# kyutai-labs/moshi

Hardware: AMD Instinct MI355X
Metric: 12.5 Hz frames/s end-to-end Mimi+Moshi-7B (higher is better)
Workload: dtype bf16

## Files before the change

### include/moshi_mi.h

```cpp
#ifndef MOSHI_MI_H_
#define MOSHI_MI_H_

#include <stdint.h>

#ifdef __cplusplus
extern "C" {
#endif

#define MMI_ABI_VERSION 3

typedef enum mmi_status {
    MMI_OK = 0,
    MMI_ERR_INVALID = -1,
    MMI_ERR_SHAPE = -2,
    MMI_ERR_STATE = -3,
    MMI_ERR_HIP = -4,
    MMI_ERR_MISSING_WEIGHT = -5,
    MMI_ERR_UNSUPPORTED = -6,
    MMI_ERR_BUSY = -7,
    MMI_ERR_NO_CHANNEL = -8
} mmi_status;

typedef enum mmi_dtype { MMI_F32 = 0, MMI_BF16 = 1, MMI_I64 = 2, MMI_F16 = 3, MMI_I8 = 4, MMI_F8E4M3 = 5 ,
                         MMI_F4E2M1X2 = 6 ,
// ... 195 lines not shown
};
typedef struct mmi_tts_script mmi_tts_script;
int mmi_lm_set_row_script(mmi_lm* lm, int32_t session, const mmi_tts_script* script, mmi_stream stream);
struct mmi_tts_status {
    int32_t has_script, end_step, n_consumed;
    int32_t* consumption_times;
    int32_t capacity;
};
typedef struct mmi_tts_status mmi_tts_status;
int mmi_lm_row_script_status(mmi_lm* lm, int32_t session, mmi_tts_status* out, mmi_stream stream);

int mmi_lm_step(mmi_lm* lm, const int64_t* user_codes, int32_t n_user, int64_t* out_tokens,
                float* opt_text_logits, float* opt_audio_logits, const float* opt_noise, int32_t batch,
                int32_t* valid, mmi_stream stream);

int mmi_lm_set_phase_callback(mmi_lm* lm, int (*fn)(void* user, mmi_stream stream), void* user);

typedef struct mmi_lm_hooks {
    int (*on_text_logits)(void* user);
    int (*on_text_token)(void* user);
    int (*on_audio_tokens)(void* user);
    void* user;
} mmi_lm_hooks;
int mmi_lm_set_hooks(mmi_lm* lm, const mmi_lm_hooks* hooks_or_null);
int mmi_lm_hook_io(mmi_lm* lm, int32_t which, int32_t write, void* buf, int64_t nbytes, mmi_stream stream);
int32_t mmi_lm_has_hooks(const mmi_lm* lm);

int mmi_lm_force_next_tokens(mmi_lm* lm, const int64_t* tokens, mmi_stream stream);

int mmi_lm_set_hidden_taps(mmi_lm* lm, int32_t on);
// ... 74 lines not shown
```

### moshi_amd/_capi.py

```python
from __future__ import annotations

import ctypes as C
import os
from pathlib import Path
from typing import Dict, Optional, Sequence

import torch

_PKG = Path(__file__).resolve().parent
DEFAULT_LIB = _PKG / "libmoshi_mi.so"

MMI_OK, MMI_ERR_INVALID, MMI_ERR_SHAPE, MMI_ERR_STATE, MMI_ERR_HIP, MMI_ERR_MISSING_WEIGHT, MMI_ERR_UNSUPPORTED, MMI_ERR_BUSY, \
    MMI_ERR_NO_CHANNEL = 0, -1, -2, -3, -4, -5, -6, -7, -8
MMI_F32, MMI_BF16, MMI_I64, MMI_F16, MMI_I8, MMI_F8E4M3, MMI_F4E2M1X2, MMI_E8M0 = 0, 1, 2, 3, 4, 5, 6, 7

_DTYPES = {torch.float32: MMI_F32, torch.bfloat16: MMI_BF16, torch.int64: MMI_I64, torch.float16: MMI_F16,
           torch.int8: MMI_I8, torch.float8_e4m3fn: MMI_F8E4M3, torch.uint8: MMI_F4E2M1X2}
MXFP4_SCALE_SUFFIX = ".weight_scale_e8m0"


class TensorDesc(C.Structure):
    _fields_ = [("name", C.c_char_p), ("data", C.c_void_p), ("dtype", C.c_int32), ("ndim", C.c_int32),
                ("shape", C.c_int64 * 4)]

# ... 135 lines not shown
    "mmi_lm_streaming_stop": (C.c_int, [_P]),
    "mmi_lm_set_exec_mask": (C.c_int, [_P, _P, _P]),
    "mmi_lm_reset": (C.c_int, [_P, _P, _P]),
    "mmi_row_sampling_check": (C.c_int, [C.POINTER(RowSampling)]),
    "mmi_lm_set_row_sampling": (C.c_int, [_P, _P, C.POINTER(RowSampling), _P]),
    "mmi_lm_clear_row_sampling": (C.c_int, [_P, _P, _P]),
    "mmi_lm_set_text_end_padding_id": (C.c_int, [_P, C.c_int32]),
    "mmi_lm_set_cross_capacity": (C.c_int, [_P, C.c_int32]),
    "mmi_lm_cross_capacity": (C.c_int, [_P]),
    "mmi_lm_set_row_condition": (C.c_int, [_P, C.c_int32, C.POINTER(RowCondition), _P]),
    "mmi_lm_enable_tts_machine": (C.c_int, [_P, C.POINTER(TTSParams), C.c_int32, C.c_int32, C.c_int32]),
    "mmi_lm_set_row_script": (C.c_int, [_P, C.c_int32, C.POINTER(TTSScriptC), _P]),
    "mmi_lm_row_script_status": (C.c_int, [_P, C.c_int32, C.POINTER(TTSStatus), _P]),
    "mmi_lm_step": (C.c_int, [_P, _P, C.c_int32, _P, _P, _P, _P, C.c_int32, C.POINTER(C.c_int32), _P]),
    "mmi_lm_force_next_tokens": (C.c_int, [_P, _P, _P]),
    "mmi_lm_set_phase_callback": (C.c_int, [_P, _P, _P]),
    "mmi_lm_set_hooks": (C.c_int, [_P, C.POINTER(LMHooks)]),
    "mmi_lm_hook_io": (C.c_int, [_P, C.c_int32, C.c_int32, _P, C.c_int64, _P]),
    "mmi_mimi_get_cfg": (C.c_int, [_P, C.POINTER(MimiCfg)]),
    "mmi_lm_get_cfg": (C.c_int, [_P, C.POINTER(LMCfg)]),
    "mmi_batcher_create": (C.c_int, [_P, _P, C.POINTER(BatcherCfg), C.POINTER(_P)]),
    "mmi_batcher_destroy": (None, [_P]),
    "mmi_batcher_open": (C.c_int, [_P, C.POINTER(C.c_int64)]),
    "mmi_batcher_open_with": (C.c_int, [_P, C.POINTER(RowSampling), C.POINTER(C.c_int64)]),
    "mmi_batcher_open_cond": (C.c_int, [_P, C.POINTER(RowSampling), C.POINTER(BatcherCondition), C.POINTER(C.c_int64)]),
    "mmi_batcher_close": (C.c_int, [_P, C.c_int64]),
    "mmi_batcher_push_pcm": (C.c_int, [_P, C.c_int64, _P, C.c_int32]),
    "mmi_batcher_step": (C.c_int, [_P, C.POINTER(C.c_int32)]),
    "mmi_batcher_pop": (C.c_int, [_P, C.c_int64, _P, _P, C.POINTER(C.c_int32)]),
    "mmi_batcher_get_stats": (C.c_int, [_P, C.POINTER(BatcherStats)]),
# ... 1 lines not shown
    "mmi_lm_launch_list": (C.c_int64, [_P, _P, C.c_int64]),
    "mmi_mimi_launch_list": (C.c_int64, [_P, C.c_int32, _P, C.c_int64]),
    "mmi_lm_seek": (C.c_int, [_P, _P, _P]),
    "mmi_lm_profile_begin": (C.c_int, [_P]),
    "mmi_lm_profile_sites": (C.c_int64, [_P, _P, C.c_int64]),
    "mmi_lm_profile_end": (C.c_int, [_P, C.POINTER(C.c_double), C.POINTER(C.c_int64), C.POINTER(C.c_int64),
                                     C.POINTER(C.c_char_p)]),
}


_SINCE_ROW_SAMPLING = ("mmi_row_sampling_check", "mmi_lm_set_row_sampling", "mmi_lm_clear_row_sampling", "mmi_batcher_open_with",
                       "mmi_lm_set_text_end_padding_id")
_SINCE_ROW_CONDITION = ("mmi_lm_set_cross_capacity", "mmi_lm_cross_capacity", "mmi_lm_set_row_condition", "mmi_batcher_open_cond")
_SINCE_TTS_MACHINE = ("mmi_lm_enable_tts_machine", "mmi_lm_set_row_script", "mmi_lm_row_script_status")
_SINCE_MANY_ROWS = ("mmi_lm_create_rows",)


def _missing(name, path):
    what = ("handles above 64 model rows" if name in _SINCE_MANY_ROWS else
            "the TTS script machine" if name in _SINCE_TTS_MACHINE else
            "per-session conditions" if name in _SINCE_ROW_CONDITION else "per-session sampling")

    def refuse(*_a):
        raise RuntimeError(f"{path} does not export {name}: it was built before {what} existed")
    return refuse


class Lib:

    def __init__(self, path: Path):
        self.path = Path(path)
        self.cdll = C.CDLL(str(self.path))
        for name, (res, args) in SIGNATURES.items():
            if name in _SINCE_ROW_SAMPLING + _SINCE_ROW_CONDITION + _SINCE_TTS_MACHINE + _SINCE_MANY_ROWS and not hasattr(self.cdll, name):
                setattr(self, name, _missing(name, self.path))
                continue
            fn = getattr(self.cdll, name)
            fn.restype = res
            fn.argtypes = args
            setattr(self, name, fn)

    def last_error(self) -> str:
        msg = self.mmi_last_error()
        return msg.decode() if msg else ""

    def check(self, rc: int) -> None:
        if rc == MMI_OK:
            return
        msg = f"{self.last_error()} (mmi status {rc})"
# ... 90 lines not shown
```

### moshi_amd/csrc/duplex.hip

```cpp
#include "mmi_common.h"

namespace {

__global__ void k_flag_publish(long* flag, long v) { mmi_flag_publish(flag, v); }
__global__ void k_flag_wait(const long* flag, long v) {
    if (threadIdx.x == 0) mmi_flag_wait(flag, v);
}

enum { S_IN = 0, S_ENC0, S_ENC1, S_WAIT0, S_WAIT1, S_LM0, S_PHASE, S_LM1, S_DEC0, S_DEC1, S_COUNT };
__global__ void k_stamp(long* p) { *p = mmi_wall_clock(); }
__global__ void k_flag_wait_stamped(const long* flag, long v, long* p) {
    if (threadIdx.x == 0) {
        p[0] = mmi_wall_clock();
        mmi_flag_wait(flag, v);
        p[1] = mmi_wall_clock();
    }
}

struct Pending { bool live = false, valid = false; float* pcm_out = nullptr; int64_t* tokens_out = nullptr; long frame = 0; };

enum { F_ENC = 0, F_LM = 1, F_DEC = 2, F_IN = 3, F_COUNT = 4 };

}

// ... 126 lines not shown
    } else {
        MMI_HIP_CHECK(hipStreamCreateWithFlags(&d->sL, hipStreamNonBlocking));
        MMI_HIP_CHECK(hipStreamCreateWithFlags(&d->sE, hipStreamNonBlocking));
        MMI_HIP_CHECK(hipStreamCreateWithFlags(&d->sD, hipStreamNonBlocking));
    }
    for (int i = 0; i < 2; ++i) {
        MMI_HIP_CHECK(hipEventCreateWithFlags(&d->ev_lm[i], hipEventDisableTiming));
        MMI_HIP_CHECK(hipEventCreateWithFlags(&d->ev_phase[i], hipEventDisableTiming));
        MMI_HIP_CHECK(hipMalloc((void**)&d->codes[i], (size_t)d->B * d->K * sizeof(int64_t)));
    }
    for (int i = 0; i < 3; ++i) {
        MMI_HIP_CHECK(hipEventCreateWithFlags(&d->ev_dec[i], hipEventDisableTiming));
        MMI_HIP_CHECK(hipMalloc((void**)&d->tokens[i], (size_t)d->B * d->NTOK * sizeof(int64_t)));
    }
    for (int i = 0; i < d->in_slots; ++i) MMI_HIP_CHECK(hipMalloc((void**)&d->pcm_in[i], (size_t)d->B * d->F * sizeof(float)));
    return MMI_OK;
}

int enqueue_decode(mmi_duplex* d, int p, bool host_saw_step) {
    Pending& q = d->pend[p];
    if (!q.live) return MMI_OK;
    int rc;
    if (!host_saw_step && (rc = await(d, F_LM, q.frame, d->sD))) return rc;
    if (d->timeline) MMI_HIP_CHECK(hipEventRecord(d->tl[6], d->sD));
    stamp(d, q.frame, S_DEC0, d->sD);
    if (q.tokens_out)
        MMI_HIP_CHECK(hipMemcpyAsync(q.tokens_out, d->tokens[p], (size_t)d->B * d->NTOK * sizeof(int64_t), hipMemcpyDeviceToDevice, d->sD));
    if (q.valid && (rc = mmi_mimi_decode_step_strided(d->mimi, d->tokens[p] + 1, d->NTOK, q.pcm_out, d->B, d->dep_q, 1, d->sD))) return rc;
    if (d->timeline) MMI_HIP_CHECK(hipEventRecord(d->tl[7], d->sD));
    stamp(d, q.frame, S_DEC1, d->sD);
// ... 166 lines not shown
```

### moshi_amd/csrc/lm_engine.hip

```cpp
#include "lm_kernels.h"
#include "mmi_graph.h"

#include <math.h>
#include <stdio.h>
#include <map>

namespace {

struct GemmW {
    u32x4* wp = nullptr;
    int N = 0, K = 0, NT = 0, KSTEPS = 0, gate = 0;
    float* scale = nullptr;
    float* scb = nullptr;
    int wq = 0;
    int ksteps = 0;
    uint8_t* s4 = nullptr;
    float xinv = 1.f;
    size_t bytes = 0;
    int T = 32;
};

struct LayerW {
    GemmW in_proj, out_proj, ffn_in, ffn_out;
    uint16_t *n1 = nullptr, *n2 = nullptr;
// ... 75 lines not shown
    bool act8 = false;
    uint8_t *xnq = nullptr, *attq = nullptr, *hbq = nullptr, *toutq = nullptr, *dxnq = nullptr;
    float *sx_xn = nullptr, *sx_tout = nullptr, *sx_dxn = nullptr, *sx_att = nullptr, *sx_hb = nullptr;
    bool hidden_taps = false;
    uint16_t* htap = nullptr;
    uint16_t *dx = nullptr, *dxn = nullptr, *dqkv = nullptr, *datt = nullptr, *dhb = nullptr, *dlogits = nullptr;
    uint16_t* dpre = nullptr;
    uint16_t *dkc = nullptr, *dvc = nullptr;
    float* noise = nullptr;
    int* use_noise = nullptr;
    int* forced = nullptr;
    int* use_forced = nullptr;
    bool forced_armed = false;
    bool noise_on = false;
    unsigned long long* rng = nullptr;
    RowSamp* rowtab = nullptr;
    int* thist = nullptr;
    std::vector<uint8_t> row_active;
    int text_eop = 0;
    mmi_lm_hooks hooks{nullptr, nullptr, nullptr, nullptr};
    bool in_hook = false;
    size_t op_text_sample = 0, op_after_text_sample = 0, op_commit = 0;
    size_t op_depformer = 0;
    int (*phase_fn)(void*, mmi_stream) = nullptr;
    void* phase_user = nullptr;
    SampleArgs text_sample_args;
    bool tts_on = false;
    TtsParams tts_p{};
    int tts_max_entries = 0, tts_max_tokens = 0, tts_max_prefix = 0;
    int tts_stride = 0;
    int* tts = nullptr;
    int* tts_stage = nullptr;
    std::vector<hipEvent_t> tts_stage_ev;
    std::vector<uint8_t> tts_stage_used;
    bool tts_rule_done = false;
    long offset_cpu = 0;
    int attn_ns = 1;
    long depth_bound = 0;
    long xlds_launches = 0;
    long rows_launches = 0;
    bool precapture_failed = false;
    bool dominant_xlds = false;
    MmiProgram prog;
    FILE* trace_file = nullptr;
    std::string trace_name;
    unsigned long long* trace_dev = nullptr;
    std::vector<unsigned long long> trace_prev;
    long trace_step = 0;
    hipStream_t cap_stream = nullptr;
    bool use_graph = true;
    struct SiteEv { size_t op; hipEvent_t ev; };
    std::vector<SiteEv> site_ev;
    size_t site_ev_used = 0;
    bool profiling = false;
    std::vector<EvPair> ev_pool;
// ... 773 lines not shown
    const int n_user = c.n_q - c.dep_q;
    MmiProgram& P = lm->prog;
    const bool a8 = lm->act8;
    P.site("prepare");
    {
        TokArgs t = tok_args(lm);
        const int* user = lm->user_i32; int* tokens = lm->tokens;
        const uint16_t *emb = lm->emb, *temb = lm->text_emb; uint16_t* x = lm->x; const int NC = lm->NC, card1 = c.card + 1;
        const int T = lm->T, xks = packed_ksteps(lm, d);
        float* rope = lm->rope; const float max_period = c.max_period;
        const int G = lm->gen_batch;
        const bool guided = lm->cfg_coef != 1.f;
        const int* masked_until = lm->masked_until; const int no_text = lm->cfg_no_text; long* offsets_m = lm->offsets_m;
        const uint16_t* cond = lm->cond;
        const uint16_t* temb2 = lm->demux ? lm->text_emb2 : nullptr; const int text_n = c.text_card + 1;
        P.add([=](hipStream_t s) {
            MMI_LAUNCH(k_lm_prepare, mmi_cdiv(G * NC + G * (Dh / 2), 128), 128, 0, s, t, user, n_user, tokens, rope, Dh, max_period);
            if (guided)
                MMI_LAUNCH(k_lm_cfg_twins, mmi_cdiv(G * NC + G * Dh + G, 128), 128, 0, s, t, tokens, masked_until, no_text, offsets_m, rope, Dh);
            if (temb2) MMI_LAUNCH(k_lm_embed_demux, dim3(mmi_cdiv(d, 256), B), 256, 0, s, (const int*)tokens, NC, emb, card1, temb, temb2,
                                  text_n, x, d, T, xks, cond);
            else MMI_LAUNCH(k_lm_embed, dim3(mmi_cdiv(d, 256), B), 256, 0, s, (const int*)tokens, NC, emb, card1, temb, x, d, T, xks, cond);
            MMI_CHECK_LAUNCH();
            return (int)MMI_OK;
        });
    }
    const int NS = attn_splits(lm->knobs, c, B);
    lm->attn_ns = NS;
    const bool kv8 = c.kv_cache_dtype == MMI_F8E4M3;
    const size_t kv_layer = (size_t)B * H * c.context * Dh / (kv8 ? 2 : 1);
    Pending pending;
    for (int l = 0; l < c.num_layers; ++l) {
// ... 181 lines not shown
            if (a8) add_q8_gemm(lm, L.ffn_out[k], lm->dhb, c.depformer_ffn_hidden, lm->dx, dd, true, MMI_EPI_RESID, lm->dx);
            else add_gemm(lm, L.ffn_out[k], lm->dhb, lm->dx, dd, true, MMI_EPI_RESID, lm->dx);
        }
        uint16_t* lg = lm->dlogits + (size_t)k * B * c.card;
        P.site("dep.lin");
        if (a8) add_q8_gemm(lm, lm->dep_lin[k], lm->dx, dd, lg, c.card, false, MMI_EPI_STORE, nullptr);
        else add_gemm(lm, lm->dep_lin[k], lm->dx, lg, c.card, false, MMI_EPI_STORE, nullptr);
        P.site("dep.sample");
        add_sample(lm, lg, c.card, c.card, false, 1 + k, lm->audio_tok + k, c.dep_q, grouped && k + 1 < c.dep_q ? k + 1 : -1);
    }
    P.site("commit");
    lm->op_commit = P.ops.size();
    {
        TokArgs t = tok_args(lm);
        const int *tt = lm->text_tok, *at = lm->audio_tok; int* out = lm->out_i32; unsigned long long* rng = lm->rng;
        P.add([=](hipStream_t s) {
            TokArgs tc = t;
            if (lm->tts_rule_done) tc.tts_audio = 0;
            MMI_LAUNCH(k_lm_commit, mmi_cdiv(tc.B, 64), 64, 0, s, tc, tt, at, out, rng);
            MMI_CHECK_LAUNCH();
            return (int)MMI_OK;
        });
    }
    return MMI_OK;
}

int project_cross_source(mmi_lm* lm, const uint16_t* src, size_t slot0, int ncol, hipStream_t s) {
    const mmi_lm_cfg& c = lm->cfg;
    const int d = c.dim, T = lm->T, ksteps = packed_ksteps(lm, d);
    const size_t slots = (size_t)lm->batch * lm->cross_cap;
    uint16_t* xp = lm->xn;
    for (int col0 = 0; col0 < ncol; col0 += T) {
        const int n = ncol - col0 < T ? ncol - col0 : T;
        MMI_HIP_CHECK(hipMemsetAsync(xp, 0, (size_t)ksteps * 512 * sizeof(uint16_t), s));
// ... 466 lines not shown
    ok &= hipSuccess == A.alloc(&lm->dkc, dkvn);
    ok &= hipSuccess == A.alloc(&lm->dvc, dkvn);
    ok &= hipSuccess == A.alloc(&lm->noise, (size_t)G * (1 + c.dep_q) * lm->kmax);
    ok &= hipSuccess == A.alloc(&lm->use_noise, (size_t)1);
    ok &= hipSuccess == A.alloc(&lm->forced, (size_t)G * (1 + c.dep_q));
    ok &= hipSuccess == A.alloc(&lm->use_forced, (size_t)1);
    ok &= hipSuccess == A.alloc(&lm->rng, (size_t)2);
    ok &= hipSuccess == A.alloc(&lm->rowtab, (size_t)G);
    ok &= hipSuccess == A.alloc(&lm->thist, (size_t)G * MMI_TEXT_HIST);
    lm->tts = nullptr;
    lm->tts_stride = 0;
    if (lm->tts_on) {
        lm->tts_stride = MMI_TTS_HDR + 2 * lm->tts_max_tokens + 3 * lm->tts_max_entries + 1 + (1 + c.dep_q) * lm->tts_max_prefix;
        ok &= hipSuccess == A.alloc(&lm->tts, (size_t)G * lm->tts_stride);
    }
    if (!ok) return fail(mmi_fail(MMI_ERR_HIP, "out of device memory (LM streaming state)"));
    MMI_HIP_CHECK(hipMemsetAsync(lm->exec, 1, G, s));
    MMI_HIP_CHECK(hipMemsetAsync(lm->offsets, 0, G * sizeof(long), s));
    if (guided) MMI_HIP_CHECK(hipMemsetAsync(lm->offsets_m, 0, B * sizeof(long), s));
    if (lm->masked_until) {
        std::vector<int> mu(G);
        for (int i = 0; i < G; ++i) mu[i] = (int)guide->cfg_is_masked_until[i];
        MMI_HIP_CHECK(hipMemcpy(lm->masked_until, mu.data(), G * sizeof(int), hipMemcpyHostToDevice));
    }
    if (lm->cond) MMI_HIP_CHECK(hipMemcpyAsync(lm->cond, guide->condition_sum, (size_t)B * d * sizeof(uint16_t), hipMemcpyDeviceToDevice, s));
    MMI_LAUNCH(k_fill_i32, mmi_cdiv(G * lm->NC * lm->CT, 256), 256, 0, s, lm->cache, -2, (long)G * lm->NC * lm->CT);
    MMI_HIP_CHECK(hipMemsetAsync(lm->kc, 0, kvn * sizeof(uint16_t), s));
    MMI_HIP_CHECK(hipMemsetAsync(lm->vc, 0, kvn * sizeof(uint16_t), s));
    MMI_HIP_CHECK(hipMemsetAsync(lm->attn_done, 0, (size_t)B * H * sizeof(unsigned), s));
    MMI_HIP_CHECK(hipMemsetAsync(lm->dkc, 0, dkvn * sizeof(uint16_t), s));
    MMI_HIP_CHECK(hipMemsetAsync(lm->dvc, 0, dkvn * sizeof(uint16_t), s));
// ... 64 lines not shown
        }
    }
    lm->streaming = true;
    return MMI_OK;
}

extern "C" int mmi_lm_streaming_stop(mmi_lm* lm) {
    MmiDeviceGuard dev_guard_(lm ? lm->device : -1);
    if (!lm) return mmi_fail(MMI_ERR_INVALID, "null handle");
    if (!lm->streaming) return MMI_OK;
    hipDeviceSynchronize();
    if (lm->trace_file) { fclose(lm->trace_file); lm->trace_file = nullptr; }
    if (lm->trace_dev) { hipFree(lm->trace_dev); lm->trace_dev = nullptr; }
    lm->prog.clear();
    lm->st.release();
    lm->tts = nullptr;
    if (lm->tts_stage) { hipHostFree(lm->tts_stage); lm->tts_stage = nullptr; }
    for (hipEvent_t e : lm->tts_stage_ev) if (e) hipEventDestroy(e);
    lm->tts_stage_ev.clear();
    lm->tts_stage_used.clear();
    lm->streaming = false;
    lm->batch = 0;
    lm->gen_batch = 0;
    lm->cfg_coef = 1.f;
    return MMI_OK;
}

extern "C" int mmi_lm_set_exec_mask(mmi_lm* lm, const uint8_t* mask, mmi_stream stream) {
    MmiDeviceGuard dev_guard_(lm ? lm->device : -1);
    if (!lm || !mask) return mmi_fail(MMI_ERR_INVALID, "null argument");
// ... 224 lines not shown
    if (!lm || !out_tokens) return mmi_fail(MMI_ERR_INVALID, "null argument");
    if (!lm->streaming)
        return mmi_fail(MMI_ERR_STATE, "You should wrap those calls with a `with lm_gen.streaming(): ...`.");
    if (!user_codes && lm->cfg.n_q > lm->cfg.dep_q) return mmi_fail(MMI_ERR_INVALID, "null argument");
    if (batch != lm->gen_batch) return mmi_fail(MMI_ERR_SHAPE, "Got a different batch size than the streaming batch");
    const mmi_lm_cfg& c = lm->cfg;
    const int need_user = c.n_q - c.dep_q;
    if (n_user < need_user) return mmi_fail(MMI_ERR_SHAPE, "not enough user tokens");
    hipStream_t s = (hipStream_t)stream;
    const int B = batch;
    if (opt_noise)
        for (uint8_t on : lm->row_active)
            if (on) return mmi_fail(MMI_ERR_UNSUPPORTED, "supplied noise is a parity aid of the handle's own sampling settings: not available while a session has settings of its own (mmi_lm_set_row_sampling)");
    if (opt_noise && lm->samp.use_sampling && (lm->samp.top_k == 0 || lm->samp.top_k_text == 0))
        return mmi_fail(MMI_ERR_UNSUPPORTED, "supplied noise is indexed by rank in the top-k: not available with top_k = 0");
    if (need_user > 0)
        MMI_LAUNCH(k_i64_to_i32, mmi_cdiv(B * need_user, 256), 256, 0, s, (const long*)user_codes, (long)n_user, lm->user_i32, B, need_user);
    if (opt_noise) {
        MMI_HIP_CHECK(hipMemcpyAsync(lm->noise, opt_noise, (size_t)B * (1 + c.dep_q) * lm->kmax * sizeof(float), hipMemcpyDeviceToDevice, s));
        MMI_HIP_CHECK(hipMemsetAsync(lm->use_noise, 1, 1, s));
        lm->noise_on = true;
    } else if (lm->noise_on) {
        MMI_HIP_CHECK(hipMemsetAsync(lm->use_noise, 0, sizeof(int), s));
        lm->noise_on = false;
    }
    MMI_CHECK_LAUNCH();
    int rc;
    lm->prog.variant = attn_variant(lm, lm->attn_ns);
    const bool hooked = lm->hooks.on_text_logits || lm->hooks.on_text_token || lm->hooks.on_audio_tokens;
    if (hooked) {
        rc = run_step_with_hooks(lm, s);
// ... 48 lines not shown
        });
    } else rc = lm->prog.run(s, lm->use_graph && !lm->profiling, lm->cap_stream);
    if (rc) return rc;
    if (lm->attn_ns > 1 && lm->use_graph && !lm->profiling && !hooked && attn_wave_kernel(lm->knobs) && !lm->knobs.no_precapture) {
        const bool split = lm->phase_fn != nullptr;
        const long counted = lm->xlds_launches;
        for (int v = 0; v < MmiProgram::NV && !lm->precapture_failed; ++v)
            if (!lm->prog.ready(v, split) && lm->prog.precapture(v, lm->cap_stream, split, lm->op_depformer) != MMI_OK) {
                lm->precapture_failed = true;
                (void)hipGetLastError();
                fprintf(stderr, "moshi_mi: the second attention step program could not be captured ahead of time (%s); it will be captured when first needed\n",
                        mmi_last_error());
            }
        lm->xlds_launches = counted;
    }
    MMI_LAUNCH(k_i32_to_i64, mmi_cdiv(B * (c.dep_q + 1), 256), 256, 0, s, (const int*)lm->out_i32, (long*)out_tokens, B * (c.dep_q + 1));
    if (opt_text_logits)
        MMI_LAUNCH(k_bf16_to_f32, (int)mmi_cdiv64((int64_t)B * c.text_card_out, 256), 256, 0, s, (const uint16_t*)lm->text_logits, opt_text_logits, (long)B * c.text_card_out);
    if (opt_audio_logits) {
        for (int k = 0; k < c.dep_q; ++k)
            for (int b = 0; b < B; ++b)
                MMI_LAUNCH(k_bf16_to_f32, mmi_cdiv(c.card, 256), 256, 0, s, (const uint16_t*)(lm->dlogits + ((size_t)k * lm->batch + b) * c.card),
                           opt_audio_logits + ((size_t)b * c.dep_q + k) * c.card, (long)c.card);
    }
    MMI_CHECK_LAUNCH();
    if (lm->forced_armed) {
        MMI_HIP_CHECK(hipMemsetAsync(lm->use_forced, 0, sizeof(int), s));
        lm->forced_armed = false;
    }
    lm->offset_cpu += 1;
    if (lm->depth_bound < (1L << 40)) lm->depth_bound += 1;
    if (valid) *valid = lm->offset_cpu > lm->max_delay ? 1 : 0;
    return MMI_OK;
}

extern "C" int mmi_lm_set_phase_callback(mmi_lm* lm, int (*fn)(void*, mmi_stream), void* user) {
    if (!lm) return mmi_fail(MMI_ERR_INVALID, "null handle");
    lm->phase_fn = fn;
    lm->phase_user = user;
    return MMI_OK;
}

extern "C" int mmi_lm_set_hooks(mmi_lm* lm, const mmi_lm_hooks* hooks) {
    MmiDeviceGuard dev_guard_(lm ? lm->device : -1);
    if (!lm) return mmi_fail(MMI_ERR_INVALID, "null handle");
    if (hooks) lm->hooks = *hooks;
    else lm->hooks = mmi_lm_hooks{nullptr, nullptr, nullptr, nullptr};
// ... 271 lines not shown
}

extern "C" int64_t mmi_lm_stat(const mmi_lm* lm, int32_t which) {
    MmiDeviceGuard dev_guard_(lm ? lm->device : -1);
    if (!lm) return -1;
    if (which == 0) return (int64_t)lm->xlds_launches;
    if (which == 1) {
        int64_t m = 0;
        for (int v = 0; v < MmiProgram::NV; ++v)
            if (lm->prog.ready(v, false) || lm->prog.ready(v, true)) m |= 1ll << v;
        return m;
    }
    if (which == 2) return (int64_t)lm->depth_bound;
    if (which == 3) return (int64_t)lm->Td;
    if (which == 4) return (int64_t)lm->rows_launches;
    return -1;
}

extern "C" int mmi_lm_profile_begin(mmi_lm* lm) {
    MmiDeviceGuard dev_guard_(lm ? lm->device : -1);
    if (!lm) return mmi_fail(MMI_ERR_INVALID, "null handle");
    lm->profiling = true;
    lm->ev_used = 0;
    lm->site_ev_used = 0;
    lm->prog.tap = [lm](size_t i, bool begin, hipStream_t s) {
        if (!begin && i + 1 != lm->prog.ops.size()) return;
        if (lm->site_ev_used == lm->site_ev.size()) {
            mmi_lm::SiteEv e{0, nullptr};
            if (hipEventCreate(&e.ev) != hipSuccess) return;
            lm->site_ev.push_back(e);
// ... 75 lines not shown
```

### moshi_amd/csrc/lm_kernels.h

```cpp
#pragma once
#include "mmi_common.h"
#include "mmi_fp4.h"

MMI_HD long mmi_xp_index(int T, int b, int k, int ksteps) {
    const int sh = T == 32 ? 4 : 5;
    const int mt = b / T, bl = b - mt * T;
    const int ks = k >> sh, kq = (k >> 3) & ((1 << (sh - 3)) - 1), e = k & 7;
    return ((((long)mt * ksteps + ks) * 64) + kq * T + bl) * 8 + e;
}
static inline int mmi_kstep(int T) { return T == 32 ? 16 : 32; }

__global__ void k_pack_w_bf16(const uint16_t* __restrict__ W, uint16_t* __restrict__ P, int N, int K, int TN, int NT,
                              int KSTEPS, int gate_hidden) {
    long idx = (long)blockIdx.x * blockDim.x + threadIdx.x;
    long total = (long)NT * KSTEPS * 512;
    if (idx >= total) return;
    int e = (int)(idx & 7);
    int lane = (int)((idx >> 3) & 63);
    long rest = idx >> 9;
    int ks = (int)(rest % KSTEPS);
    int nt = (int)(rest / KSTEPS);
    int i, kq, kstep;
    if (TN == 32) { i = lane & 31; kq = lane >> 5; kstep = 16; } else { i = lane & 15; kq = lane >> 4; kstep = 32; }
    int k = ks * kstep + 8 * kq + e;
// ... 2838 lines not shown
    const int* r = t.tts + (long)b * t.tts_stride;
    if (r[MMI_TTS_HAS] && off - dl < (long)r[MMI_TTS_APLEN]) {
        const int v = r[t.tts_aprefix + q * t.tts_max_prefix + (int)(off - dl)];
        if (v != -2) return v;
    }
    return tok;
}

__global__ void k_tts_audio_rule(TokArgs t, int* __restrict__ audio_tok) {
    const int idx = (int)(blockIdx.x * blockDim.x + threadIdx.x);
    if (idx >= t.B * t.dep_q) return;
    const int b = idx / t.dep_q, q = idx % t.dep_q;
    if (t.exec[b]) audio_tok[idx] = mmi_tts_audio_token(t, b, q, t.offsets[b], audio_tok[idx]);
}

__global__ void k_lm_prepare(TokArgs t, const int* __restrict__ user, int n_user, int* __restrict__ tokens, float* __restrict__ rope,
                             int Dh, float max_period) {
    int idx = (int)(blockIdx.x * blockDim.x + threadIdx.x);
    if (idx >= t.B * t.NC) {
        const int r = idx - t.B * t.NC;
        if (r < t.B * (Dh / 2)) {
            const int b = r / (Dh / 2), j = r - b * (Dh / 2);
            const float freq = expf((float)j * (-logf(max_period) * 2.0f / (float)Dh));
            const float ang = freq * (float)t.offsets[b];
            rope[2 * r] = cosf(ang);
            rope[2 * r + 1] = sinf(ang);
        }
        return;
    }
    const int b = idx / t.NC, c = idx % t.NC;
    const long off = t.offsets[b];
    const bool ex = t.exec[b] != 0;
    int* row = t.cache + ((long)b * t.NC + c) * t.CT;
    const int first_user = t.dep_q + 1;
    if (c >= first_user && ex) row[(int)((off + t.delays[c]) % t.CT)] = user[(long)b * n_user + (c - first_user)];
    const bool is_init = off <= (long)t.delays[c] || !ex;
    int tok = row[(int)(off % t.CT)];
    if (is_init) tok = c == 0 ? t.text_card : t.card;
    tokens[idx] = tok;
}

__global__ void k_lm_commit(TokArgs t, const int* __restrict__ text_tok, const int* __restrict__ audio_tok,
                            int* __restrict__ out, unsigned long long* __restrict__ rng) {
    int b = (int)(blockIdx.x * blockDim.x + threadIdx.x);
    if (b == 0) rng[1] += 1ull;
    if (b >= t.B) return;
    const bool ex = t.exec[b] != 0;
    const long off_new = t.offsets[b] + (ex ? 1 : 0);
    t.offsets[b] = off_new;
    const int pos = (int)(off_new % t.CT);
    int* rows = t.cache + (long)b * t.NC * t.CT;
    if (ex) {
        const int tt = text_tok[b];
        rows[pos] = tt;
        if (t.tts && t.tts_audio)
            for (int k = 0; k < t.dep_q; ++k) rows[(1 + k) * t.CT + pos] = mmi_tts_audio_token(t, b, k, off_new - 1, audio_tok[(long)b * t.dep_q + k]);
        else
        for (int k = 0; k < t.dep_q; ++k) rows[(1 + k) * t.CT + pos] = audio_tok[(long)b * t.dep_q + k];
        if (t.rows[b].active && tt != t.text_pad && tt != t.text_eop && tt != t.text_card) {
            const unsigned n = t.rows[b].hist_n;
            t.thist[(long)b * MMI_TEXT_HIST + (int)(n & (unsigned)(MMI_TEXT_HIST - 1))] = tt;
            t.rows[b].hist_n = n + 1u;
        }
    }
    const bool hide = off_new <= (long)t.max_delay || !ex;
    for (int c = 0; c <= t.dep_q; ++c) {
        long i = (off_new - t.max_delay + t.delays[c]) % t.CT;
        if (i < 0) i += t.CT;
        int v = rows[c * t.CT + (int)i];
        out[(long)b * (t.dep_q + 1) + c] = hide ? -2 : v;
    }
}

__global__ void k_i64_to_i32(const long* __restrict__ src, long src_rstride, int* __restrict__ dst, int rows, int cols) {
    int idx = (int)(blockIdx.x * blockDim.x + threadIdx.x);
    if (idx >= rows * cols) return;
    int r = idx / cols, c = idx % cols;
    dst[idx] = (int)src[(long)r * src_rstride + c];
}
__global__ void k_i32_to_i64(const int* __restrict__ src, long* __restrict__ dst, int n) {
    int idx = (int)(blockIdx.x * blockDim.x + threadIdx.x);
    if (idx < n) dst[idx] = (long)src[idx];
}
__global__ void k_bf16_to_f32(const uint16_t* __restrict__ src, float* __restrict__ dst, long n) {
    long idx = (long)blockIdx.x * blockDim.x + threadIdx.x;
// ... 103 lines not shown
```

### moshi_amd/csrc/mmi_knobs.h

```cpp
#pragma once
#include <limits.h>
#include <stdio.h>
#include <stdlib.h>
#include <atomic>
#include <string>
#include <vector>

struct MmiKnobs {
    static constexpr int UNSET = INT_MIN;

    bool no_graph = false;
    char debug_poison = 0;
    std::vector<std::string> skip_sites;

    int lm_tile = 0;
    int dep_tile = 0;
    bool no_dep_in_group = false;
    int gemm_ksplit = 0;
    bool gemm_osplit_set = false;
    int gemm_osplit = UNSET;
    bool gemm_osplit_all = false;
    char gemm_lds = 0;
    int gemm_lds_grid = UNSET;
    char gemm_once = 0;
    bool no_norm_fusion = false;
    bool q8_act_bf16 = false;
    bool q8_u2 = false;
    bool q8_tiles_serial = false;
    bool rows_groups = false;
    int rows_ntw = 0;
    bool attn_split = false;
    int attn_ns = 0;
    int attn_solo = UNSET;
    bool attn_merge_kernel = false;
    bool no_dep_attn_fusion = false;
    bool dep_attn0_launch = false;
    bool no_precapture = false;
    bool debug_trace = false;
    std::string debug_trace_prefix;
    std::string debug_dump;

    int conv_mtb = 0;
    int conv_w = 0;
    int conv_ksplit = 0;
    long res_fusion_min = UNSET;
    bool mimi_no_align = false;
    bool rvq_no_pair = false;
    bool mimi_pack_launches = false;
    bool mimi_attn_two_pass = false;
    bool mimi_two_commits = false;

    int duplex_codec_cus = 0;
// ... 53 lines not shown
    {
        const char* e = getenv("MMI_ROWS_GROUPS");
        k.rows_groups = e && e[0] && e[0] != '0';
    }
    k.rows_ntw = one_of(number("MMI_ROWS_NTW", 0), {1, 2});
    k.attn_split = first("MMI_ATTN") == 's';
    {
        const int v = number("MMI_ATTN_NS", 0);
        k.attn_ns = v >= 1 && v <= 16 ? v : 0;
    }
    k.attn_solo = number("MMI_ATTN_SOLO", MmiKnobs::UNSET);
    k.attn_merge_kernel = first("MMI_ATTN_MERGE") == 'k';
    k.no_dep_attn_fusion = present("MMI_NO_DEP_ATTN_FUSION");
    k.dep_attn0_launch = present("MMI_DEP_ATTN0_LAUNCH");
    k.no_precapture = present("MMI_NO_PRECAPTURE");
    if (const char* e = getenv("MMI_DEBUG_TRACE")) { k.debug_trace = true; k.debug_trace_prefix = e; }
    if (const char* e = getenv("MMI_DEBUG_DUMP")) k.debug_dump = e;

    k.conv_mtb = one_of(number("MMI_CONV_MTB", 0), {1, 2, 4});
    k.conv_w = one_of(number("MMI_CONV_W", 0), {1, 2, 4, 8});
    {
        const int v = number("MMI_CONV_KSPLIT", 0);
        k.conv_ksplit = v >= 1 && v <= 8 ? v : 0;
    }
    if (const char* e = getenv("MMI_MIMI_RES_FUSION_MIN")) k.res_fusion_min = atol(e);
    k.mimi_no_align = present("MMI_MIMI_NO_ALIGN");
    k.rvq_no_pair = present("MMI_RVQ_NO_PAIR");
    k.mimi_pack_launches = present("MMI_MIMI_PACK_LAUNCHES");
    k.mimi_attn_two_pass = present("MMI_MIMI_ATTN_TWO_PASS");
    k.mimi_two_commits = present("MMI_MIMI_TWO_COMMITS");
// ... 19 lines not shown
```

Before: 4465.

## Bind token I/O rings to LM and fuse prepare with embedding and commit

Adds mmi_lm_bind_io so the duplex pipeline registers its int64 code/token slot buffers with the LM. The prepare and commit kernels then read and write those slots directly through a device-side ring index, which removes the per-step i64/i32 conversion launches. The prepare kernel is also fused with the token embedding sum, and commit is parallelised across codebooks with 256-thread blocks. In exchange the ring index is tracked on both host and device, which adds state that must stay in sync, and env knobs are added to fall back to the old paths.

Result: no change. 4472 (median of 3 runs) (+0.2%).

```diff
diff --git a/include/moshi_mi.h b/include/moshi_mi.h
--- a/include/moshi_mi.h
+++ b/include/moshi_mi.h
@@ -233,6 +233,9 @@
                 float* opt_text_logits, float* opt_audio_logits, const float* opt_noise, int32_t batch,
                 int32_t* valid, mmi_stream stream);
 
+int mmi_lm_bind_io(mmi_lm* lm, const int64_t* const* codes_slots, int32_t n_in, int32_t n_user, int64_t* const* tokens_slots,
+                   int32_t n_out, mmi_stream stream);
+
 int mmi_lm_set_phase_callback(mmi_lm* lm, int (*fn)(void* user, mmi_stream stream), void* user);
 
 typedef struct mmi_lm_hooks {
diff --git a/moshi_amd/_capi.py b/moshi_amd/_capi.py
--- a/moshi_amd/_capi.py
+++ b/moshi_amd/_capi.py
@@ -173,6 +173,7 @@
     "mmi_lm_row_script_status": (C.c_int, [_P, C.c_int32, C.POINTER(TTSStatus), _P]),
     "mmi_lm_step": (C.c_int, [_P, _P, C.c_int32, _P, _P, _P, _P, C.c_int32, C.POINTER(C.c_int32), _P]),
     "mmi_lm_force_next_tokens": (C.c_int, [_P, _P, _P]),
+    "mmi_lm_bind_io": (C.c_int, [_P, _P, C.c_int32, C.c_int32, _P, C.c_int32, _P]),
     "mmi_lm_set_phase_callback": (C.c_int, [_P, _P, _P]),
     "mmi_lm_set_hooks": (C.c_int, [_P, C.POINTER(LMHooks)]),
     "mmi_lm_hook_io": (C.c_int, [_P, C.c_int32, C.c_int32, _P, C.c_int64, _P]),
@@ -204,10 +205,12 @@
 _SINCE_ROW_CONDITION = ("mmi_lm_set_cross_capacity", "mmi_lm_cross_capacity", "mmi_lm_set_row_condition", "mmi_batcher_open_cond")
 _SINCE_TTS_MACHINE = ("mmi_lm_enable_tts_machine", "mmi_lm_set_row_script", "mmi_lm_row_script_status")
 _SINCE_MANY_ROWS = ("mmi_lm_create_rows",)
+_SINCE_BIND_IO = ("mmi_lm_bind_io",)
 
 
 def _missing(name, path):
-    what = ("handles above 64 model rows" if name in _SINCE_MANY_ROWS else
+    what = ("bound token buffers" if name in _SINCE_BIND_IO else
+            "handles above 64 model rows" if name in _SINCE_MANY_ROWS else
             "the TTS script machine" if name in _SINCE_TTS_MACHINE else
             "per-session conditions" if name in _SINCE_ROW_CONDITION else "per-session sampling")
 
@@ -222,7 +225,7 @@
         self.path = Path(path)
         self.cdll = C.CDLL(str(self.path))
         for name, (res, args) in SIGNATURES.items():
-            if name in _SINCE_ROW_SAMPLING + _SINCE_ROW_CONDITION + _SINCE_TTS_MACHINE + _SINCE_MANY_ROWS and not hasattr(self.cdll, name):
+            if name in _SINCE_ROW_SAMPLING + _SINCE_ROW_CONDITION + _SINCE_TTS_MACHINE + _SINCE_MANY_ROWS + _SINCE_BIND_IO and not hasattr(self.cdll, name):
                 setattr(self, name, _missing(name, self.path))
                 continue
             fn = getattr(self.cdll, name)
diff --git a/moshi_amd/csrc/duplex.hip b/moshi_amd/csrc/duplex.hip
--- a/moshi_amd/csrc/duplex.hip
+++ b/moshi_amd/csrc/duplex.hip
@@ -164,6 +164,7 @@
         MMI_HIP_CHECK(hipMalloc((void**)&d->tokens[i], (size_t)d->B * d->NTOK * sizeof(int64_t)));
     }
     for (int i = 0; i < d->in_slots; ++i) MMI_HIP_CHECK(hipMalloc((void**)&d->pcm_in[i], (size_t)d->B * d->F * sizeof(float)));
+    if ((rc = mmi_lm_bind_io(d->lm, d->codes, 2, d->K, d->tokens, d->slots, d->sL))) return rc;
     return MMI_OK;
 }
 
diff --git a/moshi_amd/csrc/lm_engine.hip b/moshi_amd/csrc/lm_engine.hip
--- a/moshi_amd/csrc/lm_engine.hip
+++ b/moshi_amd/csrc/lm_engine.hip
@@ -113,6 +113,8 @@
     bool forced_armed = false;
     bool noise_on = false;
     unsigned long long* rng = nullptr;
+    LmIo* io = nullptr;
+    LmIo io_cpu{};
     RowSamp* rowtab = nullptr;
     int* thist = nullptr;
     std::vector<uint8_t> row_active;
@@ -138,6 +140,7 @@
     long depth_bound = 0;
     long xlds_launches = 0;
     long rows_launches = 0;
+    long conv_launches = 0;
     bool precapture_failed = false;
     bool dominant_xlds = false;
     MmiProgram prog;
@@ -941,8 +944,17 @@
         const int* masked_until = lm->masked_until; const int no_text = lm->cfg_no_text; long* offsets_m = lm->offsets_m;
         const uint16_t* cond = lm->cond;
         const uint16_t* temb2 = lm->demux ? lm->text_emb2 : nullptr; const int text_n = c.text_card + 1;
+        LmIo* io = lm->io;
+        const bool fused = !guided && !temb2 && !lm->knobs.no_prepare_fusion;
+        const int dblocks = mmi_cdiv(d, 256);
         P.add([=](hipStream_t s) {
-            MMI_LAUNCH(k_lm_prepare, mmi_cdiv(G * NC + G * (Dh / 2), 128), 128, 0, s, t, user, n_user, tokens, rope, Dh, max_period);
+            if (fused) {
+                MMI_LAUNCH(k_lm_prepare, dblocks * G + mmi_cdiv(G * NC + G * (Dh / 2), 256), 256, 0, s, t, io, user, n_user, tokens, rope, Dh,
+                           max_period, emb, card1, temb, x, d, T, xks, cond, dblocks);
+                MMI_CHECK_LAUNCH();
+                return (int)MMI_OK;
+            }
+            MMI_LAUNCH(k_lm_prepare_tokens, mmi_cdiv(G * NC + G * (Dh / 2), 128), 128, 0, s, t, io, user, n_user, tokens, rope, Dh, max_period);
             if (guided)
                 MMI_LAUNCH(k_lm_cfg_twins, mmi_cdiv(G * NC + G * Dh + G, 128), 128, 0, s, t, tokens, masked_until, no_text, offsets_m, rope, Dh);
             if (temb2) MMI_LAUNCH(k_lm_embed_demux, dim3(mmi_cdiv(d, 256), B), 256, 0, s, (const int*)tokens, NC, emb, card1, temb, temb2,
@@ -1154,10 +1166,13 @@
     {
         TokArgs t = tok_args(lm);
         const int *tt = lm->text_tok, *at = lm->audio_tok; int* out = lm->out_i32; unsigned long long* rng = lm->rng;
+        LmIo* io = lm->io;
+        const bool serial = lm->knobs.commit_serial;
         P.add([=](hipStream_t s) {
             TokArgs tc = t;
             if (lm->tts_rule_done) tc.tts_audio = 0;
-            MMI_LAUNCH(k_lm_commit, mmi_cdiv(tc.B, 64), 64, 0, s, tc, tt, at, out, rng);
+            if (serial) MMI_LAUNCH(k_lm_commit_serial, mmi_cdiv(tc.B, 64), 64, 0, s, tc, tt, at, out, rng, io);
+            else MMI_LAUNCH(k_lm_commit, mmi_cdiv(tc.B, 256 / (tc.dep_q + 1)), 256, 0, s, tc, tt, at, out, rng, io);
             MMI_CHECK_LAUNCH();
             return (int)MMI_OK;
         });
@@ -1654,7 +1669,11 @@
         lm->tts_stride = MMI_TTS_HDR + 2 * lm->tts_max_tokens + 3 * lm->tts_max_entries + 1 + (1 + c.dep_q) * lm->tts_max_prefix;
         ok &= hipSuccess == A.alloc(&lm->tts, (size_t)G * lm->tts_stride);
     }
+    ok &= hipSuccess == hipMalloc((void**)&lm->io, sizeof(LmIo));
     if (!ok) return fail(mmi_fail(MMI_ERR_HIP, "out of device memory (LM streaming state)"));
+    memset(&lm->io_cpu, 0, sizeof(LmIo));
+    lm->conv_launches = 0;
+    MMI_HIP_CHECK(hipMemsetAsync(lm->io, 0, sizeof(LmIo), s));
     MMI_HIP_CHECK(hipMemsetAsync(lm->exec, 1, G, s));
     MMI_HIP_CHECK(hipMemsetAsync(lm->offsets, 0, G * sizeof(long), s));
     if (guided) MMI_HIP_CHECK(hipMemsetAsync(lm->offsets_m, 0, B * sizeof(long), s));
@@ -1749,6 +1768,8 @@
     if (lm->trace_dev) { hipFree(lm->trace_dev); lm->trace_dev = nullptr; }
     lm->prog.clear();
     lm->st.release();
+    if (lm->io) { hipFree(lm->io); lm->io = nullptr; }
+    memset(&lm->io_cpu, 0, sizeof(LmIo));
     lm->tts = nullptr;
     if (lm->tts_stage) { hipHostFree(lm->tts_stage); lm->tts_stage = nullptr; }
     for (hipEvent_t e : lm->tts_stage_ev) if (e) hipEventDestroy(e);
@@ -2003,7 +2024,30 @@
             if (on) return mmi_fail(MMI_ERR_UNSUPPORTED, "supplied noise is a parity aid of the handle's own sampling settings: not available while a session has settings of its own (mmi_lm_set_row_sampling)");
     if (opt_noise && lm->samp.use_sampling && (lm->samp.top_k == 0 || lm->samp.top_k_text == 0))
         return mmi_fail(MMI_ERR_UNSUPPORTED, "supplied noise is indexed by rank in the top-k: not available with top_k = 0");
-    if (need_user > 0)
+    LmIo& io = lm->io_cpu;
+    int in_slot = -1, out_slot = -1;
+    if (need_user > 0 && n_user == io.in_stride)
+        for (int i = 0; i < io.n_in; ++i) if ((const long*)user_codes == io.in[i]) in_slot = i;
+    for (int i = 0; i < io.n_out; ++i) if ((long*)out_tokens == io.out[i]) out_slot = i;
+    const bool in_bound = in_slot >= 0, out_bound = out_slot >= 0;
+    if (in_bound && in_slot != io.in_next) {
+        MMI_LAUNCH(k_fill_i32, 1, 64, 0, s, &lm->io->in_next, in_slot, 1L);
+        io.in_next = in_slot;
+    }
+    if (out_bound && out_slot != io.out_next) {
+        MMI_LAUNCH(k_fill_i32, 1, 64, 0, s, &lm->io->out_next, out_slot, 1L);
+        io.out_next = out_slot;
+    }
+    if ((in_bound ? 1 : 0) != io.use_in) {
+        MMI_HIP_CHECK(hipMemsetAsync(&lm->io->use_in, in_bound ? 1 : 0, in_bound ? 1 : sizeof(int), s));
+        io.use_in = in_bound ? 1 : 0;
+    }
+    if ((out_bound ? 1 : 0) != io.use_out) {
+        MMI_HIP_CHECK(hipMemsetAsync(&lm->io->use_out, out_bound ? 1 : 0, out_bound ? 1 : sizeof(int), s));
+        io.use_out = out_bound ? 1 : 0;
+    }
+    lm->conv_launches += (need_user > 0 && !in_bound ? 1 : 0) + (out_bound ? 0 : 1);
+    if (need_user > 0 && !in_bound)
         MMI_LAUNCH(k_i64_to_i32, mmi_cdiv(B * need_user, 256), 256, 0, s, (const long*)user_codes, (long)n_user, lm->user_i32, B, need_user);
     if (opt_noise) {
         MMI_HIP_CHECK(hipMemcpyAsync(lm->noise, opt_noise, (size_t)B * (1 + c.dep_q) * lm->kmax * sizeof(float), hipMemcpyDeviceToDevice, s));
@@ -2082,7 +2126,9 @@
             }
         lm->xlds_launches = counted;
     }
-    MMI_LAUNCH(k_i32_to_i64, mmi_cdiv(B * (c.dep_q + 1), 256), 256, 0, s, (const int*)lm->out_i32, (long*)out_tokens, B * (c.dep_q + 1));
+    if (!out_bound) MMI_LAUNCH(k_i32_to_i64, mmi_cdiv(B * (c.dep_q + 1), 256), 256, 0, s, (const int*)lm->out_i32, (long*)out_tokens, B * (c.dep_q + 1));
+    if (io.n_in > 0) io.in_next = (io.in_next + 1) % io.n_in;
+    if (io.n_out > 0) io.out_next = (io.out_next + 1) % io.n_out;
     if (opt_text_logits)
         MMI_LAUNCH(k_bf16_to_f32, (int)mmi_cdiv64((int64_t)B * c.text_card_out, 256), 256, 0, s, (const uint16_t*)lm->text_logits, opt_text_logits, (long)B * c.text_card_out);
     if (opt_audio_logits) {
@@ -2099,6 +2145,31 @@
     lm->offset_cpu += 1;
     if (lm->depth_bound < (1L << 40)) lm->depth_bound += 1;
     if (valid) *valid = lm->offset_cpu > lm->max_delay ? 1 : 0;
+    return MMI_OK;
+}
+
+extern "C" int mmi_lm_bind_io(mmi_lm* lm, const int64_t* const* codes_slots, int32_t n_in, int32_t n_user, int64_t* const* tokens_slots,
+                               int32_t n_out, mmi_stream stream) {
+    MmiDeviceGuard dev_guard_(lm ? lm->device : -1);
+    if (!lm) return mmi_fail(MMI_ERR_INVALID, "null handle");
+    if (!lm->streaming) return mmi_fail(MMI_ERR_STATE, "not streaming");
+    if (n_in < 0 || n_in > MMI_IO_SLOTS || n_out < 0 || n_out > MMI_IO_SLOTS)
+        return mmi_fail(MMI_ERR_INVALID, "mmi_lm_bind_io: at most " + std::to_string(MMI_IO_SLOTS) + " slots per ring");
+    if ((n_in > 0 && !codes_slots) || (n_out > 0 && !tokens_slots)) return mmi_fail(MMI_ERR_INVALID, "null argument");
+    if (n_in > 0 && n_user < lm->cfg.n_q - lm->cfg.dep_q) return mmi_fail(MMI_ERR_SHAPE, "not enough user tokens");
+    for (int i = 0; i < n_in; ++i) if (!codes_slots[i]) return mmi_fail(MMI_ERR_INVALID, "null slot");
+    for (int i = 0; i < n_out; ++i) if (!tokens_slots[i]) return mmi_fail(MMI_ERR_INVALID, "null slot");
+    hipStream_t s = (hipStream_t)stream;
+    LmIo io;
+    memset(&io, 0, sizeof(io));
+    if (!lm->knobs.no_bind_io) {
+        for (int i = 0; i < n_in; ++i) io.in[i] = (const long*)codes_slots[i];
+        for (int i = 0; i < n_out; ++i) io.out[i] = (long*)tokens_slots[i];
+        io.n_in = n_in; io.n_out = n_out; io.in_stride = n_in > 0 ? n_user : 0;
+    }
+    MMI_HIP_CHECK(hipMemcpyAsync(lm->io, &io, sizeof(io), hipMemcpyHostToDevice, s));
+    MMI_HIP_CHECK(hipStreamSynchronize(s));
+    lm->io_cpu = io;
     return MMI_OK;
 }
 
@@ -2400,6 +2471,7 @@
     if (which == 2) return (int64_t)lm->depth_bound;
     if (which == 3) return (int64_t)lm->Td;
     if (which == 4) return (int64_t)lm->rows_launches;
+    if (which == 5) return (int64_t)lm->conv_launches;
     return -1;
 }
 
diff --git a/moshi_amd/csrc/lm_kernels.h b/moshi_amd/csrc/lm_kernels.h
--- a/moshi_amd/csrc/lm_kernels.h
+++ b/moshi_amd/csrc/lm_kernels.h
@@ -2876,9 +2876,37 @@
     if (t.exec[b]) audio_tok[idx] = mmi_tts_audio_token(t, b, q, t.offsets[b], audio_tok[idx]);
 }
 
-__global__ void k_lm_prepare(TokArgs t, const int* __restrict__ user, int n_user, int* __restrict__ tokens, float* __restrict__ rope,
-                             int Dh, float max_period) {
-    int idx = (int)(blockIdx.x * blockDim.x + threadIdx.x);
+#define MMI_IO_SLOTS 8
+struct LmIo {
+    const long* in[MMI_IO_SLOTS];
+    long* out[MMI_IO_SLOTS];
+    int n_in, n_out, in_stride;
+    int use_in, use_out;
+    int in_next, out_next;
+    int in_cur, out_cur;
+};
+
+__device__ __forceinline__ int mmi_lm_user_code(const LmIo* __restrict__ io, const int* __restrict__ user, int n_user, int b, int j) {
+    if (io->use_in) return (int)io->in[io->in_next][(long)b * io->in_stride + j];
+    return user[(long)b * n_user + j];
+}
+
+__device__ __forceinline__ int mmi_lm_input_token(const TokArgs& t, const LmIo* __restrict__ io, const int* __restrict__ user, int n_user,
+                                                  int b, int c, long off, bool ex) {
+    const int* row = t.cache + ((long)b * t.NC + c) * t.CT;
+    const int first_user = t.dep_q + 1;
+    const int dl = t.delays[c];
+    const int rd = (int)(off % t.CT);
+    int tok;
+    if (c >= first_user && ex && (int)((off + dl) % t.CT) == rd) tok = mmi_lm_user_code(io, user, n_user, b, c - first_user);
+    else tok = row[rd];
+    if (off <= (long)dl || !ex) tok = c == 0 ? t.text_card : t.card;
+    return tok;
+}
+
+__device__ __forceinline__ void mmi_lm_prepare_thread(const TokArgs& t, LmIo* __restrict__ io, const int* __restrict__ user, int n_user,
+                                                      int* __restrict__ tokens, float* __restrict__ rope, int Dh, float max_period, int idx) {
+    if (idx == 0) { io->in_cur = io->in_next; io->out_cur = io->out_next; }
     if (idx >= t.B * t.NC) {
         const int r = idx - t.B * t.NC;
         if (r < t.B * (Dh / 2)) {
@@ -2895,17 +2923,103 @@
     const bool ex = t.exec[b] != 0;
     int* row = t.cache + ((long)b * t.NC + c) * t.CT;
     const int first_user = t.dep_q + 1;
-    if (c >= first_user && ex) row[(int)((off + t.delays[c]) % t.CT)] = user[(long)b * n_user + (c - first_user)];
-    const bool is_init = off <= (long)t.delays[c] || !ex;
-    int tok = row[(int)(off % t.CT)];
-    if (is_init) tok = c == 0 ? t.text_card : t.card;
-    tokens[idx] = tok;
-}
-
-__global__ void k_lm_commit(TokArgs t, const int* __restrict__ text_tok, const int* __restrict__ audio_tok,
-                            int* __restrict__ out, unsigned long long* __restrict__ rng) {
+    if (c >= first_user && ex) row[(int)((off + t.delays[c]) % t.CT)] = mmi_lm_user_code(io, user, n_user, b, c - first_user);
+    tokens[idx] = mmi_lm_input_token(t, io, user, n_user, b, c, off, ex);
+}
+
+__global__ void k_lm_prepare_tokens(TokArgs t, LmIo* __restrict__ io, const int* __restrict__ user, int n_user, int* __restrict__ tokens,
+                             float* __restrict__ rope, int Dh, float max_period) {
+    mmi_lm_prepare_thread(t, io, user, n_user, tokens, rope, Dh, max_period, (int)(blockIdx.x * blockDim.x + threadIdx.x));
+}
+
+__global__ __launch_bounds__(256) void k_lm_prepare(TokArgs t, LmIo* __restrict__ io, const int* __restrict__ user, int n_user,
+                                                          int* __restrict__ tokens, float* __restrict__ rope, int Dh, float max_period,
+                                                          const uint16_t* __restrict__ emb, int card1, const uint16_t* __restrict__ text_emb,
+                                                          uint16_t* __restrict__ x, int D, int T, int ksteps, const uint16_t* __restrict__ cond,
+                                                          int dblocks) {
+    const int n_embed = dblocks * t.B, tid = (int)threadIdx.x;
+    if ((int)blockIdx.x >= n_embed) {
+        mmi_lm_prepare_thread(t, io, user, n_user, tokens, rope, Dh, max_period, ((int)blockIdx.x - n_embed) * 256 + tid);
+        return;
+    }
+    MMI_SHARED int tk[64];
+    const int b = (int)blockIdx.x / dblocks;
+    const int d = ((int)blockIdx.x % dblocks) * 256 + tid;
+    const int n_codebooks = t.NC;
+    if (tid < n_codebooks) tk[tid] = mmi_lm_input_token(t, io, user, n_user, b, tid, t.offsets[b], t.exec[b] != 0);
+    __syncthreads();
+    if (d >= D) return;
+    float acc = 0.f;
+    for (int c = 1; c < n_codebooks; ++c) {
+        int tok = tk[c];
+        float v = 0.f;
+        if (tok != -1) v = mmi_bf16_to_f32(emb[((long)(c - 1) * card1 + (tok < 0 ? 0 : tok)) * D + d]);
+        acc = c == 1 ? v : mmi_round_bf16(acc + v);
+    }
+    int t0 = tk[0];
+    float tv = 0.f;
+    if (t0 != -1) tv = mmi_bf16_to_f32(text_emb[(long)(t0 < 0 ? 0 : t0) * D + d]);
+    acc = n_codebooks > 1 ? mmi_round_bf16(acc + tv) : tv;
+    if (cond) acc = acc + mmi_bf16_to_f32(cond[(long)b * D + d]);
+    x[mmi_xp_index(T, b, d, ksteps)] = mmi_f32_to_bf16(acc);
+}
+
+__global__ __launch_bounds__(256) void k_lm_commit(TokArgs t, const int* __restrict__ text_tok, const int* __restrict__ audio_tok,
+                                                   int* __restrict__ out, unsigned long long* __restrict__ rng, LmIo* __restrict__ io) {
+    const int tid = (int)threadIdx.x;
+    const int W = t.dep_q + 1, spb = 256 / W;
+    if (blockIdx.x == 0 && tid == 0) {
+        rng[1] += 1ull;
+        if (io->n_in > 0) io->in_next = (io->in_cur + 1) % io->n_in;
+        if (io->n_out > 0) io->out_next = (io->out_cur + 1) % io->n_out;
+    }
+    const int bl = tid / W, c = tid - bl * W;
+    const int b = (int)blockIdx.x * spb + bl;
+    const bool live = bl < spb && b < t.B;
+    long off_old = 0;
+    bool ex = false;
+    if (live) { off_old = t.offsets[b]; ex = t.exec[b] != 0; }
+    __syncthreads();
+    if (!live) return;
+    const long off_new = off_old + (ex ? 1 : 0);
+    const int pos = (int)(off_new % t.CT);
+    int* rows = t.cache + (long)b * t.NC * t.CT;
+    int mine = 0;
+    if (c == 0) {
+        t.offsets[b] = off_new;
+        if (ex) {
+            const int tt = text_tok[b];
+            mine = tt;
+            rows[pos] = tt;
+            if (t.rows[b].active && tt != t.text_pad && tt != t.text_eop && tt != t.text_card) {
+                const unsigned n = t.rows[b].hist_n;
+                t.thist[(long)b * MMI_TEXT_HIST + (int)(n & (unsigned)(MMI_TEXT_HIST - 1))] = tt;
+                t.rows[b].hist_n = n + 1u;
+            }
+        }
+    } else if (ex) {
+        const int k = c - 1;
+        mine = audio_tok[(long)b * t.dep_q + k];
+        if (t.tts && t.tts_audio) mine = mmi_tts_audio_token(t, b, k, off_new - 1, mine);
+        rows[(long)c * t.CT + pos] = mine;
+    }
+    const bool hide = off_new <= (long)t.max_delay || !ex;
+    long i = (off_new - t.max_delay + t.delays[c]) % t.CT;
+    if (i < 0) i += t.CT;
+    int v = (ex && (int)i == pos) ? mine : rows[(long)c * t.CT + (int)i];
+    if (hide) v = -2;
+    out[(long)b * W + c] = v;
+    if (io->use_out) io->out[io->out_cur][(long)b * W + c] = (long)v;
+}
+
+__global__ void k_lm_commit_serial(TokArgs t, const int* __restrict__ text_tok, const int* __restrict__ audio_tok,
+                                   int* __restrict__ out, unsigned long long* __restrict__ rng, LmIo* __restrict__ io) {
     int b = (int)(blockIdx.x * blockDim.x + threadIdx.x);
-    if (b == 0) rng[1] += 1ull;
+    if (b == 0) {
+        rng[1] += 1ull;
+        if (io->n_in > 0) io->in_next = (io->in_cur + 1) % io->n_in;
+        if (io->n_out > 0) io->out_next = (io->out_cur + 1) % io->n_out;
+    }
     if (b >= t.B) return;
     const bool ex = t.exec[b] != 0;
     const long off_new = t.offsets[b] + (ex ? 1 : 0);
@@ -2926,11 +3040,13 @@
         }
     }
     const bool hide = off_new <= (long)t.max_delay || !ex;
+    long* out64 = io->use_out ? io->out[io->out_cur] : nullptr;
     for (int c = 0; c <= t.dep_q; ++c) {
         long i = (off_new - t.max_delay + t.delays[c]) % t.CT;
         if (i < 0) i += t.CT;
-        int v = rows[c * t.CT + (int)i];
-        out[(long)b * (t.dep_q + 1) + c] = hide ? -2 : v;
+        const int v = hide ? -2 : rows[c * t.CT + (int)i];
+        out[(long)b * (t.dep_q + 1) + c] = v;
+        if (out64) out64[(long)b * (t.dep_q + 1) + c] = (long)v;
     }
 }
 
diff --git a/moshi_amd/csrc/mmi_knobs.h b/moshi_amd/csrc/mmi_knobs.h
--- a/moshi_amd/csrc/mmi_knobs.h
+++ b/moshi_amd/csrc/mmi_knobs.h
@@ -36,6 +36,9 @@
     bool no_dep_attn_fusion = false;
     bool dep_attn0_launch = false;
     bool no_precapture = false;
+    bool no_bind_io = false;
+    bool no_prepare_fusion = false;
+    bool commit_serial = false;
     bool debug_trace = false;
     std::string debug_trace_prefix;
     std::string debug_dump;
@@ -119,6 +122,9 @@
     k.no_dep_attn_fusion = present("MMI_NO_DEP_ATTN_FUSION");
     k.dep_attn0_launch = present("MMI_DEP_ATTN0_LAUNCH");
     k.no_precapture = present("MMI_NO_PRECAPTURE");
+    k.no_bind_io = present("MMI_NO_BIND_IO");
+    k.no_prepare_fusion = present("MMI_NO_PREPARE_FUSION");
+    k.commit_serial = first("MMI_COMMIT") == 's';
     if (const char* e = getenv("MMI_DEBUG_TRACE")) { k.debug_trace = true; k.debug_trace_prefix = e; }
     if (const char* e = getenv("MMI_DEBUG_DUMP")) k.debug_dump = e;
 
```
